# edwardyehuang/iSeg

Hardware: AMD Instinct MI355X
Metric: train_images_per_sec (ConvNeXt-T+ASPP 512x512 crop, fwd+bwd+AdamW, whole job) (higher is better)
Workload: dtype bf16

## Files before the change

### include/iseg_hip.h

```cpp
#ifndef ISEG_HIP_H
#define ISEG_HIP_H

#include <stddef.h>
#include <stdint.h>

#ifdef __cplusplus
extern "C" {
#endif

#ifndef ISEG_HIP_STREAM_T
#define ISEG_HIP_STREAM_T
typedef struct ihipStream_t* iseg_stream_t;
#endif

#define ISEG_STATUS_OK 0
#define ISEG_STATUS_ARG (-1)
#define ISEG_STATUS_HIP (-2)
#define ISEG_STATUS_UNSUPPORTED (-3)
#define ISEG_STATUS_WORKSPACE (-4)

#define ISEG_DTYPE_F32 0
#define ISEG_DTYPE_BF16 1

#define ISEG_ACT_NONE 0
// ... 524 lines not shown

size_t iseg_convnext_mlp_bwd_data_ln_workspace_bytes(int64_t M, int C);
int iseg_convnext_mlp_bwd_data_ln(const void* y1, const float* mean, const float* rstd, const float* ln_gamma, const float* ln_beta,
                                  const void* dout, const float* rowscale, int64_t rows_per_group, const void* bw_tiled, const float* b1,
                                  void* dy1, float* dln_gamma, float* dln_beta, int64_t M, int C, int dtype, void* ws, size_t ws_bytes,
                                  iseg_stream_t stream);
int iseg_convnext_mlp_fwd_ln(const void* y1, const float* ln_gamma, const float* ln_beta, float eps, float* mean, float* rstd,
                             const void* fw_tiled, const float* b1, const float* b2, const float* gamma, const float* rowscale,
                             int64_t rows_per_group, const void* residual, void* out, int64_t M, int C, int dtype, iseg_stream_t stream);
size_t iseg_convnext_mlp_wgrad_workspace_bytes(int64_t M, int C);
int iseg_convnext_mlp_wgrad(const void* y, const float* mean, const float* rstd, const float* ln_gamma, const float* ln_beta,
                            const void* dout, const float* rowscale, int64_t rows_per_group, const void* bw_tiled, const float* b1,
                            const float* W2, const float* b2, const float* gamma, float* dW1, float* db1, float* dW2, float* db2,
                            float* dgamma, int64_t M, int C, int dtype, void* ws, size_t ws_bytes, iseg_stream_t stream);

int iseg_gemma_rope(const void* qkv, int64_t ld_in, void* out, int64_t ld_out, const float* table, int64_t rows, int T, int nq, int nkv, int h,
                    int inverse, int dtype, iseg_stream_t stream);
int iseg_gemma_attention_supported(int nq, int nkv, int h, int dtype);
size_t iseg_gemma_attention_lse_elems(int64_t batch, int T, int nq, int nkv);
int iseg_gemma_attention_fwd(const void* q, int64_t ldq, const void* k, int64_t ldk, const void* v, int64_t ldv, const uint8_t* padding_mask,
                             void* out, int64_t ldo, float* lse2, int64_t batch, int T, int nq, int nkv, int h, float scale, int dtype,
                             iseg_stream_t stream);
int iseg_gemma_attention_bwd(const void* q, int64_t ldq, const void* k, int64_t ldk, const void* v, int64_t ldv, const uint8_t* padding_mask,
                             const void* out, int64_t ldo, const void* dout, int64_t lddo, const float* lse2, float* dsum, void* dq,
                             int64_t lddq, void* dk, int64_t lddk, void* dv, int64_t lddv, int64_t batch, int T, int nq, int nkv, int h,
                             float scale, int dtype, iseg_stream_t stream);
int iseg_embedding_grad(const void* dy, const int64_t* sorted_ids, const int64_t* order, float* dtable, int64_t n, int64_t vocab, int d,
                        float scale, int dtype, iseg_stream_t stream);
int iseg_gemma_rope_cache(const void* qkv, int64_t ld_in, void* q_out, int64_t ldq, void* kcache, int64_t k_batch, int64_t ldk, void* vcache,
                          int64_t v_batch, int64_t ldv, const float* table, int64_t batch, int S, int pos0, int Tn, int nq, int nkv, int h,
// ... 43 lines not shown
```

### iseg_amd/_hip.py

```python
import ctypes as C
import os

_HERE = os.path.dirname(os.path.abspath(__file__))
LIB_PATH = os.path.join(_HERE, "lib", "libiseg_hip.so")

F32, BF16 = 0, 1
ACT_NONE, ACT_RELU, ACT_GELU, ACT_GELU_GRAD, ACT_RELU_GRAD, ACT_MUL_AUX, ACT_SIGMOID, ACT_SWISH, ACT_GELU_TANH = 0, 1, 2, 3, 4, 5, 6, 7, 8
SAMPLE_RANDOM, SAMPLE_TOP_K, SAMPLE_TOP_P = 0, 1, 2
IDS_I32, IDS_I64 = 0, 1


class HipLibraryMissing(RuntimeError):
    pass


class HipCallError(RuntimeError):
    pass


class GemmArgs(C.Structure):
    _fields_ = [
        ("A", C.c_void_p), ("lda", C.c_int64), ("a_kcontig", C.c_int),
        ("B", C.c_void_p), ("ldb", C.c_int64), ("b_kcontig", C.c_int),
        ("D", C.c_void_p), ("ldd", C.c_int64),
# ... 249 lines not shown
    "iseg_conv2d_branches_fwd": (_i, [_p, C.POINTER(ConvBranches), _i, _p, _z, _p]),
    "iseg_conv2d_branches_bwd_data": (_i, [C.POINTER(ConvBranches), _p, _p, _l, _i, _p, _z, _p]),
    "iseg_conv2d_branches_bwd_weight": (_i, [_p, C.POINTER(ConvBranches), _i, _i, _p, _z, _p]),
    "iseg_convnext_mlp_supported": (_i, [_i, _i]),
    "iseg_convnext_mlp_tiled_bytes": (_z, [_i, _i]),
    "iseg_convnext_mlp_prep": (_i, [_p, _p, _p, _p, _p, _i, _p]),
    "iseg_convnext_mlp_fwd": (_i, [_p, _p, _p, _p, _p, _p, _l, _p, _p, _l, _i, _i, _p]),
    "iseg_convnext_mlp_bwd": (_i, [_p, _p, _p, _p, _p, _p, _p, _l, _i, _i, _p]),
    "iseg_convnext_mlp_bwd_data": (_i, [_p, _p, _p, _p, _p, _p, _p, _l, _p, _p, _p, _l, _i, _i, _p]),
    "iseg_convnext_mlp_bwd_data_ln_workspace_bytes": (_z, [_l, _i]),
    "iseg_convnext_mlp_bwd_data_ln": (_i, [_p, _p, _p, _p, _p, _p, _p, _l, _p, _p, _p, _p, _p, _l, _i, _i, _p, _z, _p]),
    "iseg_convnext_weight_prep_batched": (_i, [_p, _i, _l, _p]),
    "iseg_convnext_mlp_fwd_ln": (_i, [_p, _p, _p, _f, _p, _p, _p, _p, _p, _p, _p, _l, _p, _p, _l, _i, _i, _p]),
    "iseg_convnext_mlp_wgrad_workspace_bytes": (_z, [_l, _i]),
    "iseg_convnext_mlp_wgrad": (_i, [_p, _p, _p, _p, _p, _p, _p, _l, _p, _p, _p, _p, _p, _p, _p, _p, _p, _p, _l, _i, _i, _p, _z, _p]),
    "iseg_gemma_rope": (_i, [_p, _l, _p, _l, _p, _l, _i, _i, _i, _i, _i, _i, _p]),
    "iseg_gemma_attention_supported": (_i, [_i, _i, _i, _i]),
    "iseg_gemma_attention_lse_elems": (_z, [_l, _i, _i, _i]),
    "iseg_gemma_attention_fwd": (_i, [_p, _l, _p, _l, _p, _l, _p, _p, _l, _p, _l, _i, _i, _i, _i, _f, _i, _p]),
    "iseg_gemma_attention_bwd": (_i, [_p, _l, _p, _l, _p, _l, _p, _p, _l, _p, _l, _p, _p, _p, _l, _p, _l, _p, _l, _l, _i, _i, _i, _i, _f, _i, _p]),
    "iseg_embedding_grad": (_i, [_p, _p, _p, _p, _l, _l, _i, _f, _i, _p]),
    "iseg_gemma_rope_cache": (_i, [_p, _l, _p, _l, _p, _l, _l, _p, _l, _l, _p, _l, _i, _i, _i, _i, _i, _i, _i, _p]),
    "iseg_gemma_decode_attention_supported": (_i, [_i, _i, _i, _i, _i]),
    "iseg_gemma_decode_attention_splits": (_i, [_l, _i, _i, _i, _i, _i]),
    "iseg_gemma_decode_attention_scratch_bytes": (_z, [_l, _i, _i, _i, _i, _i, _i]),
    "iseg_gemma_decode_attention": (_i, [_p, _l, _p, _l, _l, _p, _l, _l, _p, _l, _p, _z, _l, _i, _i, _i, _i, _i, _i, _f, _i, _i, _p]),
    "iseg_gemma_rope_cache_at": (_i, [_p, _l, _p, _l, _p, _l, _l, _p, _l, _l, _p, _l, _i, _p, _i, _i, _i, _i, _i, _p]),
    "iseg_gemma_decode_attention_at": (_i, [_p, _l, _p, _l, _l, _p, _l, _l, _p, _l, _p, _z, _l, _i, _p, _i, _i, _i, _i, _f, _i, _i, _p]),
    "iseg_decode_commit": (_i, [_p, _l, _p, _l, _p, _p, _p, _p, _l, _i, _l, _i, _i, _p]),
    "iseg_token_sample_supported": (_i, [_l, _i, _i, _i]),
# ... 47 lines not shown
```

### iseg_amd/build.py

```python
import os
import subprocess
import sys
from concurrent.futures import ThreadPoolExecutor

HERE = os.path.dirname(os.path.abspath(__file__))
ROOT = os.path.dirname(HERE)
CSRC = os.path.join(HERE, "csrc")
LIBDIR = os.path.join(HERE, "lib")
LIB = os.path.join(LIBDIR, "libiseg_hip.so")
SOURCES = ["api.hip", "gemm.hip", "gemm_nn.hip", "gemm_nt.hip", "gemm_tn.hip", "norm.hip", "dwconv.hip", "dwconv_mfma.hip", "dwconv_wgrad_mfma.hip", "dwconv_strided.hip", "elementwise.hip", "resize.hip", "loss.hip", "confusion.hip", "ohem.hip", "mask_loss.hip", "sod_metrics.hip", "sod_fmv2.hip", "ccl.hip", "optim.hip", "misc.hip", "attention.hip", "dcnv3.hip", "defattn.hip", "winattn.hip", "flashattn.hip", "selfattn.hip", "mlp_fused.hip", "mlp_wgrad.hip", "conv_igemm.hip", "conv_patchify.hip", "augment.hip", "projective.hip", "grn.hip", "eva.hip", "comm.hip", "mbconv.hip", "sepconv.hip", "jpu.hip", "resblock.hip", "gemma.hip", "gemma_decode.hip", "decode_commit.hip", "token_sample.hip", "lm_head_ce.hip"]
FLAGS = ["--offload-arch=gfx950", "-O3", "-fPIC", "-std=c++17", "-I" + os.path.join(ROOT, "include"), "-I" + CSRC,
         "-Wno-unused-result"] + [f"-D{d}" for d in os.environ.get("ISEG_BUILD_DEFINES", "").split() if d]


def _hipcc():
    for c in (os.environ.get("HIPCC"), "/opt/rocm/bin/hipcc", "hipcc"):
        if c and (os.path.isabs(c) and os.path.exists(c) or not os.path.isabs(c)):
            return c
    raise RuntimeError("hipcc not found")


def _stale(out, deps):
    if not os.path.exists(out):
        return True
    t = os.path.getmtime(out)
# ... 34 lines not shown
```

### iseg_amd/csrc/mlp_wgrad.hip

```cpp
#include "common.h"
#include "iseg_hip.h"
#include "mlp_common.h"

namespace {

typedef __attribute__((address_space(3))) bf16x4* lds_bf16x4_ptr;

template <int C> struct WgGeom {
    static constexpr int WAVES = 8, NT = 64 * WAVES, RT = C > 96 ? 32 : 64;
    static constexpr int HID = 4 * C, KS = C / 32, CBS = C / 16;
    static constexpr int NHG = HID / (16 * WAVES);
    static constexpr int STRIDE = (((2 * C + 223) / 256) * 256 + 32) / 2;
    static constexpr int TILE = RT * STRIDE;
    static constexpr int CPR = C / 8;
    static constexpr int RG = (NT / CPR) >= 32 ? 32 : 16;
    static constexpr int NLOAD = CPR * RG, RPT = RT / RG;
    static constexpr int LDS = 2 * 2 * TILE * 2;
    static constexpr int IMG = C * 64, SLAB = 3 * IMG;
    static_assert(C % 32 == 0 && HID % (16 * WAVES) == 0 && NLOAD <= NT && RT % RG == 0 && LDS <= 160 * 1024, "geometry");
};

__device__ __forceinline__ f32x4 mfma16(const bf16x8& a, const bf16x8& b, const f32x4& c) {
    return __builtin_amdgcn_mfma_f32_16x16x32_bf16(a, b, c, 0, 0, 0);
}

__device__ __forceinline__ bf16x8 tr_frag(const bf16_t* rows, int stride, int cb, int lane) {
    const int q = lane >> 4, qq = (lane >> 2) & 3, p = lane & 3;
    const bf16_t* a0 = rows + (4 * q + qq) * stride + 16 * cb + 4 * p;
    const bf16x4 lo = __builtin_amdgcn_ds_read_tr16_b64_v4bf16((lds_bf16x4_ptr)(a0));
    const bf16x4 hi = __builtin_amdgcn_ds_read_tr16_b64_v4bf16((lds_bf16x4_ptr)(a0 + 16 * stride));
    bf16x8 f;
#pragma unroll
    for (int i = 0; i < 4; ++i) {
        f[i] = lo[i];
        f[4 + i] = hi[i];
    }
    return f;
}

template <int C>
__global__ __launch_bounds__(512) void convnext_mlp_wgrad_kernel(const bf16_t* __restrict__ Y, const float* __restrict__ mean,
                                                                 const float* __restrict__ rstd, const float* __restrict__ ln_gamma,
                                                                 const float* __restrict__ ln_beta, const bf16_t* __restrict__ D,
                                                                 const float* __restrict__ rowscale, int64_t rows_per_group,
                                                                 const void* __restrict__ BW, const float* __restrict__ b1,
                                                                 float* __restrict__ part, int64_t M, int64_t rows_per_chunk, int nchunk) {
    using G = WgGeom<C>;
    constexpr int HID = G::HID, KS = G::KS, CBS = G::CBS, STRIDE = G::STRIDE, TILE = G::TILE, RT = G::RT, RG = G::RG, RPT = G::RPT, CPR = G::CPR;
    extern __shared__ __attribute__((aligned(16))) char smem[];
    bf16_t* const tiles = reinterpret_cast<bf16_t*>(smem);

    const int wg = blockIdx.x, xcd = wg & 7, idx = wg >> 3;
    const int hg = idx % G::NHG, chunk = (idx / G::NHG) * 8 + xcd;
    if (chunk >= nchunk) return;
// ... 196 lines not shown
        v = __builtin_bit_cast(float, (unsigned)sx[0]) + __builtin_bit_cast(float, (unsigned)sx[1]);
        if (lane < 16) pb[hid0 + li] = v;
    }
    if (hg == 0) {
        float* const ss = reinterpret_cast<float*>(smem);
        if (loader) {
#pragma unroll
            for (int u = 0; u < 8; ++u) ss[rg * C + 8 * cpos + u] = s_acc[u];
        }
        __syncthreads();
        if (tid < C) {
            float v = 0.f;
            for (int g = 0; g < RG; ++g) v += ss[g * C + tid];
            ps[tid] = v;
        }
    }
}

constexpr int FIN_ROWS = 8;
__global__ __launch_bounds__(256) void convnext_mlp_wgrad_finish_kernel(const float* __restrict__ rec, const float* __restrict__ W2,
                                                                        const float* __restrict__ b2, const float* __restrict__ gamma,
                                                                        float* __restrict__ dW1, float* __restrict__ db1,
                                                                        float* __restrict__ dW2, float* __restrict__ db2,
                                                                        float* __restrict__ gpart, int C) {
    __shared__ float tw[FIN_ROWS][33];
    __shared__ float tg[8][32];
    const int HID = 4 * C;
    const int c0 = blockIdx.x * 32, h0 = blockIdx.y * FIN_ROWS;
    const int tx = threadIdx.x & 31, ty = threadIdx.x >> 5;
    const int c = c0 + tx;
    const int64_t plane = (int64_t)HID * C;
    const float gm = gamma ? gamma[c] : 1.f;
    {
        const int64_t o = (int64_t)(h0 + ty) * C + c;
        const float z = rec[o], w = rec[plane + o];
        dW2[o] += z * gm;
        tg[ty][tx] = W2[o] * z;
        tw[ty][tx] = w;
    }
    __syncthreads();
    {
        const int hx = threadIdx.x & (FIN_ROWS - 1), cc = threadIdx.x / FIN_ROWS;
        dW1[(int64_t)(c0 + cc) * HID + h0 + hx] += tw[hx][cc];
    }
    if (ty == 0) {
        float v = 0.f;
#pragma unroll
        for (int j = 0; j < 8; ++j) v += tg[j][tx];
        if (blockIdx.y == 0) {
            const float s = rec[2 * plane + HID + c];
            if (gamma) {
                v += b2[c] * s;
                db2[c] += gm * s;
            } else {
                db2[c] += s;
            }
        }
        if (gamma) gpart[(int64_t)blockIdx.y * C + c] = v;
    }
    if (blockIdx.x == 0 && threadIdx.x < FIN_ROWS) {
        const int hid = h0 + threadIdx.x;
        db1[hid] += rec[2 * plane + hid];
    }
}

template <int C> int rows_per_chunk_for(int64_t M, int* nchunk) {
    using G = WgGeom<C>;
    const int target = 8 * (32 / G::NHG);
    int64_t rpc = (M + target - 1) / target;
    rpc = (rpc + 63) / 64 * 64;
    if (rpc < 256) rpc = 256;
    *nchunk = (int)((M + rpc - 1) / rpc);
    return (int)rpc;
}

template <int C>
int launch_wgrad(const void* y, const float* mean, const float* rstd, const float* lng, const float* lnb, const void* d, const float* rowscale,
// ... 14 lines not shown
}

size_t wgrad_ws_floats(int C, int64_t M, int* nchunk_out) {
    int nchunk;
    if (C == 96) rows_per_chunk_for<96>(M, &nchunk);
    else rows_per_chunk_for<192>(M, &nchunk);
    if (nchunk_out) *nchunk_out = nchunk;
    const size_t rec = 2 * 4 * (size_t)C * C + 4 * C + C;
    return (size_t)(nchunk + 1) * rec + (size_t)(4 * C / FIN_ROWS) * C;
}

}

extern "C" size_t iseg_convnext_mlp_wgrad_workspace_bytes(int64_t M, int C) {
    if (!(C == 96 || C == 192) || M <= 0) return 0;
    return wgrad_ws_floats(C, M, nullptr) * sizeof(float);
}

extern "C" int iseg_convnext_mlp_wgrad(const void* y, const float* mean, const float* rstd, const float* ln_gamma, const float* ln_beta,
                                       const void* dout, const float* rowscale, int64_t rows_per_group, const void* bw_tiled, const float* b1,
                                       const float* W2, const float* b2, const float* gamma, float* dW1, float* db1, float* dW2, float* db2,
                                       float* dgamma, int64_t M, int C, int dtype, void* ws, size_t ws_bytes, hipStream_t stream) {
    ISEG_REQUIRE(dtype == ISEG_BF16 && (C == 96 || C == 192), "iseg_convnext_mlp_wgrad: bf16 storage with C = 96 or 192 only (C = %d, dtype = %d)", C, dtype);
    ISEG_REQUIRE(y && dout && bw_tiled && b1 && W2 && b2 && dW1 && db1 && dW2 && db2 && M > 0, "iseg_convnext_mlp_wgrad: null operand or empty problem");
    ISEG_REQUIRE(!gamma || dgamma, "iseg_convnext_mlp_wgrad: gamma needs dgamma");
    ISEG_REQUIRE(!mean || (rstd && ln_gamma && ln_beta), "iseg_convnext_mlp_wgrad: mean needs rstd, ln_gamma and ln_beta");
    ISEG_REQUIRE(!rowscale || (rows_per_group > 0 && rows_per_group % 64 == 0),
                 "iseg_convnext_mlp_wgrad: the row factor must be constant inside 64-row tiles (rows_per_group = %lld)", (long long)rows_per_group);
    ISEG_REQUIRE((((uintptr_t)y | (uintptr_t)dout | (uintptr_t)bw_tiled | (uintptr_t)ln_gamma | (uintptr_t)ln_beta) & 15) == 0,
                 "iseg_convnext_mlp_wgrad: operands must be 16-byte aligned");
    int nchunk;
    const size_t need = wgrad_ws_floats(C, M, &nchunk) * sizeof(float);
    ISEG_NEED_WORKSPACE("iseg_convnext_mlp_wgrad", ws, ws_bytes, need);
    float* const wsf = (float*)ws;
    int rc = C == 96 ? launch_wgrad<96>(y, mean, rstd, ln_gamma, ln_beta, dout, rowscale, rows_per_group, bw_tiled, b1, wsf, M, stream)
                     : launch_wgrad<192>(y, mean, rstd, ln_gamma, ln_beta, dout, rowscale, rows_per_group, bw_tiled, b1, wsf, M, stream);
    if (rc != ISEG_OK) return rc;
    const int HID = 4 * C;
    const int64_t rec = 2 * (int64_t)HID * C + HID + C;
    float* part = wsf;
    float* sum = part + (int64_t)nchunk * rec;
    float* gpart_ws = sum + rec;
    launch_reduce_rows(part, nchunk, rec, 0, 1, rec, sum, nullptr, rec, 0, 1.f, 0, stream);
    const int P = HID / FIN_ROWS;
    float* gpart = gpart_ws;
    float* arena = nullptr;
    if (gamma) {
// ... 12 lines not shown
```

### iseg_amd/functional.py

```python
import math
import os

import torch
from torch.autograd import Function

from . import kernels as K
from . import nn
from . import dist


def _grad(p):
    if p.grad is None:
        p.grad = torch.zeros_like(p.data)
    return p.grad


def _param_grad(p, *shape, scratch=False):
    if p is not None and p.requires_grad:
        g = _grad(p)
    elif p is None or not scratch:
        return None
    else:
        g = torch.zeros(p.shape, dtype=torch.float32, device=p.device)
    return g.reshape(shape) if shape else g
# ... 239 lines not shown
        rpg = M // rowscale.shape[0] if rowscale is not None else 0
        fw, bw = nn.mlp_tiled(W1, W2, None)
        out, mean, rstd = K.convnext_mlp_fwd_ln(x2, ln_gamma.data, ln_beta.data, eps, fw, b1.data, b2.data, None, rowscale, rpg, x2)
        ctx.params, ctx.rpg = (ln_gamma, ln_beta, W1, b1, W2, b2), rpg
        ctx.save_for_backward(x2, mean, rstd, bw, rowscale)
        return out.reshape(x.shape)

    @staticmethod
    def backward(ctx, dout):
        x2, mean, rstd, bw, rowscale = ctx.saved_tensors
        ln_gamma, ln_beta, W1, b1, W2, b2 = ctx.params
        M, C = x2.shape
        do2 = _c(dout).reshape(M, C)
        ln = (mean, rstd, ln_gamma.data, ln_beta.data)
        dx = None
        if ctx.needs_input_grad[0]:
            dln = K.convnext_mlp_bwd_data_ln(x2, do2, bw, b1.data, ln, _grad_out(ln_gamma), _grad_out(ln_beta), rowscale, ctx.rpg)
            dx = K.axpby(do2, dln, 1.0, 1.0, out=dln).reshape(dout.shape)
        else:
            K.convnext_mlp_bwd_data_ln(x2, do2, bw, b1.data, ln, _grad_out(ln_gamma), _grad_out(ln_beta), rowscale, ctx.rpg)
        if any(p.requires_grad for p in (W1, b1, W2, b2)):
            K.convnext_mlp_wgrad(x2, do2, bw, b1.data, W2.data, b2.data, None, _grad_out(W1), _grad_out(b1), _grad_out(W2), _grad_out(b2), None, rowscale,
                                 ctx.rpg, ln=ln)
        dist.grads_ready(ln_gamma, ln_beta, W1, b1, W2, b2)
        return (dx,) + (None,) * 8


def ln_mlp_residual_supported(x, params, drop_path_mask=None):
    ln_gamma, ln_beta, W1, b1, W2, b2 = params
    C = x.shape[-1]
# ... 1253 lines not shown
        ctx.p, ctx.dil, ctx.pad = p, dil, pad
        ctx.save_for_backward(xc, y1, y2, mean, rstd, h, g if grad else None, dp_mask)
        return out.reshape(N, H, W, C)

    @staticmethod
    def backward(ctx, dout):
        xc, y1, y2, mean, rstd, h, g, dp_mask = ctx.saved_tensors
        p, dil, pad = ctx.p, ctx.dil, ctx.pad
        N, H, W, C = xc.shape
        M = N * H * W
        Kk = p.dw_kernel.shape[0]
        do2 = _c(dout).reshape(M, C)
        cdt = xc.dtype
        if ctx.ln_on_load:
            y1m, ln = y1.reshape(M, C), (mean, rstd, p.ln_gamma.data, p.ln_beta.data)
            dy1 = K.convnext_mlp_bwd_data_ln(y1m, do2, h, p.b1.data, ln, _grad_out(p.ln_gamma), _grad_out(p.ln_beta), dp_mask, H * W)
            if any(q is not None and q.requires_grad for q in (p.w1, p.b1, p.w2, p.b2, p.gamma)):
                K.convnext_mlp_wgrad(y1m, do2, h, p.b1.data, p.w2.data, p.b2.data, p.gamma.data if p.gamma is not None else None,
                                     _grad_out(p.w1), _grad_out(p.b1), _grad_out(p.w2), _grad_out(p.b2),
                                     _grad_out(p.gamma) if p.gamma is not None else None, dp_mask, H * W, ln=ln)
            del h
        else:
            dy2 = _ConvNeXtBlockFn._mlp_backward_with_hidden(ctx, p, do2, y2, h, g, dp_mask, H, W, C, M, cdt, xc)
            del h, g
            dy1 = K.layernorm_bwd(dy2, y1.reshape(M, C), p.ln_gamma.data, mean, rstd, _grad_out(p.ln_gamma), _grad_out(p.ln_beta))
        dy1 = dy1.reshape(N, H, W, C)
        if p.dw_kernel.requires_grad or p.dw_bias.requires_grad:
            K.dwconv2d_bwd_weight(xc, dy1, _grad_out(p.dw_kernel, Kk * Kk, C), _grad_out(p.dw_bias), Kk, dil, pad, pad)
        dx = None
        if ctx.needs_input_grad[0]:
            padb = (Kk - 1) * dil - pad
            dx = K.dwconv2d(dy1, p.dw_kernel.data.reshape(Kk * Kk, C), None, Kk, dil, padb, padb, flip=True, add=_c(dout))
# ... 1750 lines not shown
```

### iseg_amd/kernels.py

```python
import contextlib
import ctypes as C

import torch

from . import _hip
from ._hip import F32, BF16, ACT_NONE, ACT_RELU, ACT_GELU, ACT_GELU_GRAD, ACT_RELU_GRAD, ACT_MUL_AUX, ACT_SIGMOID, ACT_SWISH, ACT_GELU_TANH, GemmArgs

_DT = {torch.float32: F32, torch.bfloat16: BF16}


def dt(t):
    try:
        return _DT[t.dtype if isinstance(t, torch.Tensor) else t]
    except KeyError:
        raise TypeError(f"iseg_amd kernels support float32 and bfloat16 storage, got {t.dtype if isinstance(t, torch.Tensor) else t}")


def ptr(t):
    return None if t is None else t.data_ptr()


_DEVICE_INDEX = [None]


# ... 304 lines not shown
    ws, wsb = workspace(need, y1.device)
    _hip.call("iseg_convnext_mlp_bwd_data_ln", ptr(y1), ptr(mean), ptr(rstd), ptr(lng), ptr(lnb), ptr(dout), ptr(rowscale), int(rows_per_group),
              ptr(bw_tiled), ptr(b1), ptr(dy1), ptr(dln_gamma), ptr(dln_beta), M, Cc, dt(y1), ptr(ws), wsb, stream())
    return dy1


def convnext_mlp_wgrad(y, dout, bw_tiled, b1, W2, b2, gamma, dW1, db1, dW2, db2, dgamma, rowscale=None, rows_per_group=0, ln=None):
    _require_cuda(y, dout, bw_tiled)
    M, Cc = y.shape
    need = _hip.lib().iseg_convnext_mlp_wgrad_workspace_bytes(M, Cc)
    ws, wsb = workspace(need, y.device)
    mean, rstd, lng, lnb = ln if ln is not None else (None, None, None, None)
    _hip.call("iseg_convnext_mlp_wgrad", ptr(y), ptr(mean), ptr(rstd), ptr(lng), ptr(lnb), ptr(dout), ptr(rowscale), int(rows_per_group),
              ptr(bw_tiled), ptr(b1), ptr(W2), ptr(b2), ptr(gamma), ptr(dW1), ptr(db1), ptr(dW2), ptr(db2), ptr(dgamma), M, Cc, dt(y), ptr(ws),
              wsb, stream())


def layernorm_fwd(x2d, gamma, beta, eps, save_stats=True):
    _require_cuda(x2d)
    rows, Cc = x2d.shape
    y = torch.empty_like(x2d)
    mean = torch.empty(rows, dtype=torch.float32, device=x2d.device) if save_stats else None
    rstd = torch.empty(rows, dtype=torch.float32, device=x2d.device) if save_stats else None
    _hip.call("iseg_layernorm_fwd", ptr(x2d), ptr(gamma), ptr(beta), ptr(y), ptr(mean), ptr(rstd), rows, Cc, eps, dt(x2d), stream())
    return y, mean, rstd


def layernorm_bwd(dy2d, x2d, gamma, mean, rstd, dgamma, dbeta, dx_add=None, accumulate=True):
    rows, Cc = x2d.shape
    dx = torch.empty_like(x2d)
# ... 1853 lines not shown
```

Baseline: 2103.

## Fuse ConvNeXt MLP data-grad, LayerNorm backward and weight-grad into one pass

Adds a single backward kernel for the C=96 bf16 ConvNeXt MLP. Each row tile is loaded once and the kernel recomputes the hidden activations, produces the input gradient through LayerNorm backward, and accumulates per-chunk W1/W2/bias/LN-parameter partials, which a finish kernel then reduces. Previously the data-grad and weight-grad kernels each re-read the activations and redid the first GEMM. The cost is a large LDS footprint and heavy register use per block, and the path only covers the first stage (C=96).

```diff
diff --git a/include/iseg_hip.h b/include/iseg_hip.h
--- a/include/iseg_hip.h
+++ b/include/iseg_hip.h
@@ -562,6 +562,12 @@
                             const float* W2, const float* b2, const float* gamma, float* dW1, float* db1, float* dW2, float* db2,
                             float* dgamma, int64_t M, int C, int dtype, void* ws, size_t ws_bytes, iseg_stream_t stream);
 
+int iseg_convnext_mlp_bwd_onepass(const void* y1, const float* mean, const float* rstd, const float* ln_gamma, const float* ln_beta,
+                                  const void* dout, const float* rowscale, int64_t rows_per_group, const void* bw_tiled, const float* b1,
+                                  const float* W2, const float* b2, const float* gamma, void* dy1, float* dln_gamma, float* dln_beta,
+                                  float* dW1, float* db1, float* dW2, float* db2, float* dgamma, int64_t M, int C, int dtype, void* ws,
+                                  size_t ws_bytes, iseg_stream_t stream);
+
 int iseg_gemma_rope(const void* qkv, int64_t ld_in, void* out, int64_t ld_out, const float* table, int64_t rows, int T, int nq, int nkv, int h,
                     int inverse, int dtype, iseg_stream_t stream);
 int iseg_gemma_attention_supported(int nq, int nkv, int h, int dtype);
diff --git a/iseg_amd/_hip.py b/iseg_amd/_hip.py
--- a/iseg_amd/_hip.py
+++ b/iseg_amd/_hip.py
@@ -287,6 +287,7 @@
     "iseg_convnext_mlp_fwd_ln": (_i, [_p, _p, _p, _f, _p, _p, _p, _p, _p, _p, _p, _l, _p, _p, _l, _i, _i, _p]),
     "iseg_convnext_mlp_wgrad_workspace_bytes": (_z, [_l, _i]),
     "iseg_convnext_mlp_wgrad": (_i, [_p, _p, _p, _p, _p, _p, _p, _l, _p, _p, _p, _p, _p, _p, _p, _p, _p, _p, _l, _i, _i, _p, _z, _p]),
+    "iseg_convnext_mlp_bwd_onepass": (_i, [_p] * 7 + [_l] + [_p] * 13 + [_l, _i, _i, _p, _z, _p]),
     "iseg_gemma_rope": (_i, [_p, _l, _p, _l, _p, _l, _i, _i, _i, _i, _i, _i, _p]),
     "iseg_gemma_attention_supported": (_i, [_i, _i, _i, _i]),
     "iseg_gemma_attention_lse_elems": (_z, [_l, _i, _i, _i]),
diff --git a/iseg_amd/build.py b/iseg_amd/build.py
--- a/iseg_amd/build.py
+++ b/iseg_amd/build.py
@@ -8,7 +8,7 @@
 CSRC = os.path.join(HERE, "csrc")
 LIBDIR = os.path.join(HERE, "lib")
 LIB = os.path.join(LIBDIR, "libiseg_hip.so")
-SOURCES = ["api.hip", "gemm.hip", "gemm_nn.hip", "gemm_nt.hip", "gemm_tn.hip", "norm.hip", "dwconv.hip", "dwconv_mfma.hip", "dwconv_wgrad_mfma.hip", "dwconv_strided.hip", "elementwise.hip", "resize.hip", "loss.hip", "confusion.hip", "ohem.hip", "mask_loss.hip", "sod_metrics.hip", "sod_fmv2.hip", "ccl.hip", "optim.hip", "misc.hip", "attention.hip", "dcnv3.hip", "defattn.hip", "winattn.hip", "flashattn.hip", "selfattn.hip", "mlp_fused.hip", "mlp_wgrad.hip", "conv_igemm.hip", "conv_patchify.hip", "augment.hip", "projective.hip", "grn.hip", "eva.hip", "comm.hip", "mbconv.hip", "sepconv.hip", "jpu.hip", "resblock.hip", "gemma.hip", "gemma_decode.hip", "decode_commit.hip", "token_sample.hip", "lm_head_ce.hip"]
+SOURCES = ["api.hip", "gemm.hip", "gemm_nn.hip", "gemm_nt.hip", "gemm_tn.hip", "norm.hip", "dwconv.hip", "dwconv_mfma.hip", "dwconv_wgrad_mfma.hip", "dwconv_strided.hip", "elementwise.hip", "resize.hip", "loss.hip", "confusion.hip", "ohem.hip", "mask_loss.hip", "sod_metrics.hip", "sod_fmv2.hip", "ccl.hip", "optim.hip", "misc.hip", "attention.hip", "dcnv3.hip", "defattn.hip", "winattn.hip", "flashattn.hip", "selfattn.hip", "mlp_fused.hip", "mlp_wgrad.hip", "mlp_bwd_onepass.hip", "conv_igemm.hip", "conv_patchify.hip", "augment.hip", "projective.hip", "grn.hip", "eva.hip", "comm.hip", "mbconv.hip", "sepconv.hip", "jpu.hip", "resblock.hip", "gemma.hip", "gemma_decode.hip", "decode_commit.hip", "token_sample.hip", "lm_head_ce.hip"]
 FLAGS = ["--offload-arch=gfx950", "-O3", "-fPIC", "-std=c++17", "-I" + os.path.join(ROOT, "include"), "-I" + CSRC,
          "-Wno-unused-result"] + [f"-D{d}" for d in os.environ.get("ISEG_BUILD_DEFINES", "").split() if d]
 
diff --git a/iseg_amd/csrc/mlp_bwd_onepass.hip b/iseg_amd/csrc/mlp_bwd_onepass.hip
--- /dev/null
+++ b/iseg_amd/csrc/mlp_bwd_onepass.hip
@@ -0,0 +1,401 @@
+#include "common.h"
+#include "iseg_hip.h"
+#include "mlp_common.h"
+#include "mlp_wgrad_common.h"
+
+namespace {
+
+struct OpGeom {
+    static constexpr int C = 96, HID = 4 * C, WAVES = 8, NT = 64 * WAVES, RT = 32, KS = C / 32, CBS = C / 16;
+    static constexpr int NG = HID / (16 * WAVES);
+    static constexpr int YSTR = 144, TILE = RT * YSTR;
+    static constexpr int WSTR = 112;
+    static constexpr int HSTR = HID + 8;
+    static constexpr int DSTR = C + 4;
+    static constexpr int CPR = C / 8, NLOAD = CPR * RT;
+    static constexpr int OFF_W1 = 2 * 2 * TILE * 2;
+    static constexpr int OFF_DH = OFF_W1 + HID * WSTR * 2;
+    static constexpr int OFF_RAW = OFF_DH + RT * HSTR * 2;
+    static constexpr int OFF_ST = OFF_RAW + 2 * RT * C * 2;
+    static constexpr int OFF_LG = OFF_ST + 2 * RT * 2 * 4;
+    static constexpr int LDS = OFF_LG + C * 4;
+    static constexpr int IMG = C * 64, SLAB = 3 * IMG;
+    static constexpr int64_t REC = 2 * (int64_t)HID * C + HID + C;
+    static_assert(NG == 3 && NLOAD <= NT && RT * DSTR * 4 <= 2 * TILE * 2 && 3 * (NT / 32) * C * 4 <= RT * HSTR * 2 && LDS <= 160 * 1024,
+                  "geometry");
+};
+
+__global__ __launch_bounds__(512) void convnext_mlp_bwd_onepass_kernel(const bf16_t* __restrict__ Y, const float* __restrict__ mean,
+                                                                       const float* __restrict__ rstd, const float* __restrict__ ln_gamma,
+                                                                       const float* __restrict__ ln_beta, const bf16_t* __restrict__ D,
+                                                                       const float* __restrict__ rowscale, int64_t rows_per_group,
+                                                                       const void* __restrict__ BW, const float* __restrict__ b1,
+                                                                       bf16_t* __restrict__ DY, float* __restrict__ part,
+                                                                       float* __restrict__ lnpart, int64_t M, int64_t rows_per_chunk) {
+    using G = OpGeom;
+    constexpr int C = G::C, HID = G::HID, KS = G::KS, CBS = G::CBS, NG = G::NG, RT = G::RT, CPR = G::CPR;
+    constexpr int YSTR = G::YSTR, TILE = G::TILE, WSTR = G::WSTR, HSTR = G::HSTR, DSTR = G::DSTR;
+    extern __shared__ __attribute__((aligned(16))) char smem[];
+    bf16_t* const tiles = reinterpret_cast<bf16_t*>(smem);
+    bf16_t* const w1img = reinterpret_cast<bf16_t*>(smem + G::OFF_W1);
+    bf16_t* const dht = reinterpret_cast<bf16_t*>(smem + G::OFF_DH);
+    bf16_t* const raws = reinterpret_cast<bf16_t*>(smem + G::OFF_RAW);
+    float* const stats = reinterpret_cast<float*>(smem + G::OFF_ST);
+    float* const lgs = reinterpret_cast<float*>(smem + G::OFF_LG);
+
+    const int chunk = blockIdx.x;
+    const int tid = threadIdx.x, wid = __builtin_amdgcn_readfirstlane(tid >> 6);
+    auto opaque = [](int v) {
+        asm volatile("" : "+v"(v));
+        return v;
+    };
+    const int64_t r_begin = (int64_t)chunk * rows_per_chunk;
+    const int64_t r_end = r_begin + rows_per_chunk < M ? r_begin + rows_per_chunk : M;
+    const int ntiles = (int)((r_end - r_begin + RT - 1) / RT);
+
+    for (int i = tid; i < HID * CPR; i += G::NT) {
+        const int hid = i / CPR, c8 = i % CPR;
+        const char* src = (const char*)BW + (int64_t)(hid >> 5) * G::SLAB + (c8 >> 1) * 1024 + mlp_frag_offset(hid & 31, c8 & 1);
+        *reinterpret_cast<bf16x8*>(w1img + hid * WSTR + 8 * c8) = *reinterpret_cast<const bf16x8*>(src);
+    }
+    if (tid < C) lgs[tid] = ln_gamma[tid];
+
+    bf16x8 ry, rd;
+    float rmean, rrstd;
+    bool rok;
+    auto issue = [&](int t) {
+        const int tq = opaque(tid);
+        const bool loader = tq < G::NLOAD;
+        const int cpos = tq % CPR, rg = loader ? tq / CPR : 0;
+        const bool live = t < ntiles;
+        const int tt = live ? t : ntiles - 1;
+        const int64_t row = r_begin + (int64_t)tt * RT + rg;
+        const int64_t rr = row < r_end ? row : r_begin;
+        ry = *reinterpret_cast<const bf16x8*>(Y + rr * C + 8 * cpos);
+        rd = *reinterpret_cast<const bf16x8*>(D + rr * C + 8 * cpos);
+        rmean = mean[rr];
+        rrstd = rstd[rr];
+        rok = live && loader && row < r_end;
+    };
+    auto commit = [&](int t, int buf) {
+        const int tq = opaque(tid);
+        const bool loader = tq < G::NLOAD;
+        const int cpos = tq % CPR, rg = loader ? tq / CPR : 0;
+        const int64_t row0 = r_begin + (int64_t)(t < ntiles ? t : ntiles - 1) * RT;
+        const float rs = rowscale ? rowscale[row0 / rows_per_group] : 1.f;
+        float lg[8], lb[8];
+        const int cp = 8 * cpos;
+        load8<float>(ln_gamma + cp, lg);
+        load8<float>(ln_beta + cp, lb);
+        bf16x8 yr = ry, y = ry, d = rd;
+        float mu = rmean, rsd = rrstd;
+        if (!rok) {
+#pragma unroll
+            for (int u = 0; u < 8; ++u) {
+                yr[u] = (bf16_t)0.f;
+                y[u] = (bf16_t)0.f;
+                d[u] = (bf16_t)0.f;
+            }
+            mu = 0.f;
+            rsd = 0.f;
+        } else {
+#pragma unroll
+            for (int u = 0; u < 8; ++u) y[u] = (bf16_t)iseg_ln_apply((float)y[u], mu, rsd, lg[u], lb[u]);
+        }
+        if (rowscale) {
+#pragma unroll
+            for (int u = 0; u < 8; ++u) d[u] = (bf16_t)((float)d[u] * rs);
+        }
+        if (loader) {
+            *reinterpret_cast<bf16x8*>(tiles + (buf * 2 + 0) * TILE + rg * YSTR + 8 * cpos) = y;
+            *reinterpret_cast<bf16x8*>(tiles + (buf * 2 + 1) * TILE + rg * YSTR + 8 * cpos) = d;
+            *reinterpret_cast<bf16x8*>(raws + (buf * RT + rg) * C + 8 * cpos) = yr;
+            if (cpos == 0) {
+                stats[(buf * RT + rg) * 2] = mu;
+                stats[(buf * RT + rg) * 2 + 1] = rsd;
+            }
+        }
+    };
+
+    f32x4 zacc[NG][CBS], wacc[NG][CBS];
+    float db1[NG];
+#pragma unroll
+    for (int g = 0; g < NG; ++g) {
+        db1[g] = 0.f;
+#pragma unroll
+        for (int cb = 0; cb < CBS; ++cb)
+#pragma unroll
+            for (int r = 0; r < 4; ++r) zacc[g][cb][r] = wacc[g][cb][r] = 0.f;
+    }
+
+    float cgs[3], cbs[3], ssum[3];
+#pragma unroll
+    for (int i = 0; i < 3; ++i) cgs[i] = cbs[i] = ssum[i] = 0.f;
+
+    constexpr int CG = 2;
+    bf16x8 w3f[KS];
+    float bias;
+    auto fetch_w3 = [&](int hg) {
+        const int lane = opaque(tid) & 63, li = lane & 15, q = lane >> 4;
+        const char* p = (const char*)BW + (hg >> 1) * G::SLAB + (hg & 1) * 256 + G::IMG + (q >> 1) * 1024 + mlp_frag_offset(li, q & 1);
+#pragma unroll
+        for (int ks = 0; ks < KS; ++ks) w3f[ks] = *reinterpret_cast<const bf16x8*>(p + ks * 2048);
+        bias = b1[hg * 16 + li];
+    };
+    fetch_w3(wid * NG);
+    auto hidden = [&](int t, int buf) {
+        const bf16_t* const ty = tiles + (buf * 2 + 0) * TILE;
+        const bf16_t* const td = tiles + (buf * 2 + 1) * TILE;
+        issue(t + 1);
+#pragma unroll
+        for (int g = 0; g < NG; ++g) {
+            const int hg = wid * NG + g, hid0 = hg * 16;
+            const int lane = opaque(tid) & 63, li = lane & 15, q = lane >> 4;
+            f32x4 hacc[2], dacc[2];
+#pragma unroll
+            for (int b = 0; b < 2; ++b)
+#pragma unroll
+                for (int r = 0; r < 4; ++r) {
+                    hacc[b][r] = bias;
+                    dacc[b][r] = 0.f;
+                }
+#pragma unroll
+            for (int ks = 0; ks < KS; ++ks) {
+                bf16x8 ay[2], ad[2];
+#pragma unroll
+                for (int b = 0; b < 2; ++b) {
+                    const int o = (b * 16 + li) * YSTR + 32 * ks + 8 * q;
+                    ay[b] = *reinterpret_cast<const bf16x8*>(ty + o);
+                    ad[b] = *reinterpret_cast<const bf16x8*>(td + o);
+                }
+                const bf16x8 w1f = *reinterpret_cast<const bf16x8*>(w1img + (hid0 + li) * WSTR + 32 * ks + 8 * q);
+                __builtin_amdgcn_sched_barrier(0);
+#pragma unroll
+                for (int b = 0; b < 2; ++b) {
+                    hacc[b] = mfma16(ay[b], w1f, hacc[b]);
+                    dacc[b] = mfma16(ad[b], w3f[ks], dacc[b]);
+                }
+                __builtin_amdgcn_sched_barrier(0);
+            }
+            fetch_w3(wid * NG + (g + 1) % NG);
+            __builtin_amdgcn_sched_barrier(0);
+            bf16x8 bd[CG], by[CG], gf, hf;
+#pragma unroll
+            for (int b = 0; b < 2; ++b) {
+#pragma unroll
+                for (int r = 0; r < 4; ++r) {
+                    float gl, gd;
+                    gelu_sig_both(hacc[b][r], gl, gd);
+                    const bf16_t dh = (bf16_t)(dacc[b][r] * gd);
+                    gf[4 * b + r] = (bf16_t)gl;
+                    hf[4 * b + r] = dh;
+                    db1[g] += (float)dh;
+                    dht[(16 * b + 4 * q + r) * HSTR + hid0 + li] = dh;
+                }
+                asm volatile("" : "+v"(db1[g]));
+                __builtin_amdgcn_sched_barrier(0);
+                if (b == 0) {
+#pragma unroll
+                    for (int c = 0; c < CG; ++c) {
+                        bd[c] = tr_frag(td, YSTR, c, lane);
+                        by[c] = tr_frag(ty, YSTR, c, lane);
+                    }
+                    __builtin_amdgcn_sched_barrier(0);
+                }
+            }
+#pragma unroll
+            for (int c0 = 0; c0 < CBS; c0 += CG) {
+                if (c0 > 0) {
+#pragma unroll
+                    for (int c = 0; c < CG; ++c) {
+                        bd[c] = tr_frag(td, YSTR, c0 + c, lane);
+                        by[c] = tr_frag(ty, YSTR, c0 + c, lane);
+                    }
+                    __builtin_amdgcn_sched_barrier(0);
+                }
+#pragma unroll
+                for (int c = 0; c < CG; ++c) {
+                    zacc[g][c0 + c] = mfma16(gf, bd[c], zacc[g][c0 + c]);
+                    wacc[g][c0 + c] = mfma16(hf, by[c], wacc[g][c0 + c]);
+                }
+                __builtin_amdgcn_sched_barrier(0);
+            }
+        }
+        const int tq = opaque(tid), hw = tq >> 5, j32 = tq & 31;
+#pragma unroll
+        for (int ps = 0; ps < 2; ++ps)
+#pragma unroll
+            for (int i = 0; i < 3; ++i) ssum[i] += (float)td[(hw + 16 * ps) * YSTR + j32 + 32 * i];
+    };
+
+    auto dy2_tile = [&](int tile, float* dyt) {
+        const int mt = tile & 1, ct = tile >> 1;
+        const int lane = opaque(tid) & 63, li = lane & 15, q = lane >> 4;
+        f32x4 acc;
+#pragma unroll
+        for (int r = 0; r < 4; ++r) acc[r] = 0.f;
+        const bf16_t* const arow = dht + (16 * mt + li) * HSTR + 4 * q;
+#pragma unroll
+        for (int ks = 0; ks < HID / 32; ++ks) {
+            const bf16x4 lo = *reinterpret_cast<const bf16x4*>(arow + 32 * ks);
+            const bf16x4 hi = *reinterpret_cast<const bf16x4*>(arow + 32 * ks + 16);
+            bf16x8 a;
+#pragma unroll
+            for (int i = 0; i < 4; ++i) {
+                a[i] = lo[i];
+                a[4 + i] = hi[i];
+            }
+            acc = mfma16(a, tr_frag(w1img + 32 * ks * WSTR, WSTR, ct, lane), acc);
+            if (ks % 4 == 3) __builtin_amdgcn_sched_barrier(0);
+        }
+#pragma unroll
+        for (int r = 0; r < 4; ++r) dyt[(16 * mt + 4 * q + r) * DSTR + 16 * ct + li] = acc[r];
+    };
+
+    auto layernorm_bwd = [&](int t, int buf, const float* dyt) {
+        const int64_t row0 = r_begin + (int64_t)t * RT;
+        const int tq = opaque(tid), hw = tq >> 5, j32 = tq & 31;
+#pragma unroll
+        for (int ps = 0; ps < 2; ++ps) {
+            const int rr = hw + 16 * ps;
+            const float mu = stats[(buf * RT + rr) * 2], rsd = stats[(buf * RT + rr) * 2 + 1];
+            float v[3], xh[3], tt[3];
+            float s1 = 0.f, s2 = 0.f;
+#pragma unroll
+            for (int i = 0; i < 3; ++i) {
+                v[i] = dyt[rr * DSTR + j32 + 32 * i];
+                xh[i] = ((float)raws[(buf * RT + rr) * C + j32 + 32 * i] - mu) * rsd;
+                tt[i] = v[i] * lgs[j32 + 32 * i];
+                s1 += tt[i];
+                s2 = fmaf(tt[i], xh[i], s2);
+            }
+#pragma unroll
+            for (int o = 16; o > 0; o >>= 1) {
+                s1 += __shfl_xor(s1, o);
+                s2 += __shfl_xor(s2, o);
+            }
+            s1 *= 1.f / (float)C;
+            s2 *= 1.f / (float)C;
+            const int64_t row = row0 + rr;
+            if (row < r_end) {
+#pragma unroll
+                for (int i = 0; i < 3; ++i) DY[row * C + j32 + 32 * i] = (bf16_t)(rsd * (tt[i] - s1 - xh[i] * s2));
+            }
+#pragma unroll
+            for (int i = 0; i < 3; ++i) {
+                cgs[i] = fmaf(v[i], xh[i], cgs[i]);
+                cbs[i] += v[i];
+            }
+        }
+    };
+
+    issue(0);
+    commit(0, 0);
+    __syncthreads();
+    for (int t = 0; t < ntiles; ++t) {
+        const int buf = t & 1;
+        hidden(t, buf);
+        __syncthreads();
+        float* const dyt = reinterpret_cast<float*>(tiles + buf * 2 * TILE);
+        dy2_tile(wid, dyt);
+        if (wid < 4) dy2_tile(8 + wid, dyt);
+        __syncthreads();
+        layernorm_bwd(t, buf, dyt);
+        commit(t + 1, buf ^ 1);
+        __syncthreads();
+    }
+
+    const int lane = tid & 63, li = lane & 15, q = lane >> 4, hw = tid >> 5, j32 = tid & 31;
+    float* const pz = part + (int64_t)chunk * G::REC;
+    float* const pw = pz + (int64_t)HID * C;
+    float* const pb = pw + (int64_t)HID * C;
+    float* const ps = pb + HID;
+#pragma unroll
+    for (int g = 0; g < NG; ++g) {
+        const int hid0 = (wid * NG + g) * 16;
+#pragma unroll
+        for (int cb = 0; cb < CBS; ++cb)
+#pragma unroll
+            for (int r = 0; r < 4; ++r) {
+                const int64_t o = (int64_t)(hid0 + 4 * q + r) * C + 16 * cb + li;
+                pz[o] = zacc[g][cb][r];
+                pw[o] = wacc[g][cb][r];
+            }
+        unsigned u = __builtin_bit_cast(unsigned, db1[g]);
+        auto sw = __builtin_amdgcn_permlane16_swap(u, u, false, false);
+        float v = __builtin_bit_cast(float, (unsigned)sw[0]) + __builtin_bit_cast(float, (unsigned)sw[1]);
+        u = __builtin_bit_cast(unsigned, v);
+        auto sx = __builtin_amdgcn_permlane32_swap(u, u, false, false);
+        v = __builtin_bit_cast(float, (unsigned)sx[0]) + __builtin_bit_cast(float, (unsigned)sx[1]);
+        if (lane < 16) pb[hid0 + li] = v;
+    }
+    float* const ls = reinterpret_cast<float*>(smem + G::OFF_DH);
+#pragma unroll
+    for (int i = 0; i < 3; ++i) {
+        ls[hw * 3 * C + j32 + 32 * i] = ssum[i];
+        ls[hw * 3 * C + C + j32 + 32 * i] = cgs[i];
+        ls[hw * 3 * C + 2 * C + j32 + 32 * i] = cbs[i];
+    }
+    __syncthreads();
+    if (tid < 3 * C) {
+        float v = 0.f;
+        for (int g = 0; g < G::NT / 32; ++g) v += ls[g * 3 * C + tid];
+        if (tid < C) ps[tid] = v;
+        else lnpart[(int64_t)chunk * 2 * C + tid - C] = v;
+    }
+}
+
+}
+
+extern "C" int iseg_convnext_mlp_bwd_onepass(const void* y1, const float* mean, const float* rstd, const float* ln_gamma, const float* ln_beta,
+                                             const void* dout, const float* rowscale, int64_t rows_per_group, const void* bw_tiled,
+                                             const float* b1, const float* W2, const float* b2, const float* gamma, void* dy1,
+                                             float* dln_gamma, float* dln_beta, float* dW1, float* db1, float* dW2, float* db2, float* dgamma,
+                                             int64_t M, int C, int dtype, void* ws, size_t ws_bytes, hipStream_t stream) {
+    using G = OpGeom;
+    ISEG_REQUIRE(dtype == ISEG_BF16 && C == 96, "iseg_convnext_mlp_bwd_onepass: bf16 storage with C = 96 only (C = %d, dtype = %d)", C, dtype);
+    ISEG_REQUIRE(y1 && mean && rstd && ln_gamma && ln_beta && dout && bw_tiled && b1 && W2 && b2 && dy1 && dln_gamma && dln_beta && dW1 && db1 &&
+                     dW2 && db2 && M > 0, "iseg_convnext_mlp_bwd_onepass: null operand or empty problem");
+    ISEG_REQUIRE(!gamma || dgamma, "iseg_convnext_mlp_bwd_onepass: gamma needs dgamma");
+    ISEG_REQUIRE(!rowscale || (rows_per_group > 0 && rows_per_group % 64 == 0),
+                 "iseg_convnext_mlp_bwd_onepass: the row factor must be constant inside 64-row tiles (rows_per_group = %lld)", (long long)rows_per_group);
+    ISEG_REQUIRE((((uintptr_t)y1 | (uintptr_t)dout | (uintptr_t)bw_tiled | (uintptr_t)ln_gamma | (uintptr_t)ln_beta | (uintptr_t)dy1) & 15) == 0,
+                 "iseg_convnext_mlp_bwd_onepass: operands must be 16-byte aligned");
+    int nchunk;
+    const size_t need = iseg_convnext_mlp_wgrad_workspace_bytes(M, C);
+    static_assert(G::REC == 2 * 4 * 96 * 96 + 4 * 96 + 96, "record of onepass_ws_floats");
+    ISEG_NEED_WORKSPACE("iseg_convnext_mlp_bwd_onepass", ws, ws_bytes, need);
+    const int rpc = onepass_rows_per_chunk(M, &nchunk);
+    float* const part = (float*)ws;
+    float* const sum = part + (int64_t)nchunk * G::REC;
+    float* const gpart_ws = sum + G::REC;
+    float* lnpart = gpart_ws + (G::HID / FIN_ROWS) * G::C;
+    float* const ln_arena = iseg_deferred_partials((size_t)nchunk * 2 * G::C * sizeof(float), dln_gamma, dln_beta, 1, stream);
+    if (ln_arena) lnpart = ln_arena;
+    static const bool raised = [] {
+        return hipFuncSetAttribute(reinterpret_cast<const void*>(&convnext_mlp_bwd_onepass_kernel), hipFuncAttributeMaxDynamicSharedMemorySize,
+                                   G::LDS) == hipSuccess;
+    }();
+    (void)raised;
+    hipLaunchKernelGGL(convnext_mlp_bwd_onepass_kernel, dim3(nchunk), dim3(G::NT), G::LDS, stream, (const bf16_t*)y1, mean, rstd, ln_gamma, ln_beta,
+                       (const bf16_t*)dout, rowscale, rows_per_group, bw_tiled, b1, (bf16_t*)dy1, part, lnpart, M, (int64_t)rpc);
+    const int rc = iseg_check_launch("iseg_convnext_mlp_bwd_onepass");
+    if (rc != ISEG_OK) return rc;
+    if (ln_arena) iseg_deferred_push(lnpart, nchunk, 2 * G::C, 2 * G::C, dln_gamma, dln_beta, G::C, 1.f, stream);
+    else launch_reduce_rows(lnpart, nchunk, 2 * G::C, 0, 1, 2 * G::C, dln_gamma, dln_beta, G::C, 0, 1.f, 1, stream);
+    launch_reduce_rows(part, nchunk, G::REC, 0, 1, G::REC, sum, nullptr, G::REC, 0, 1.f, 0, stream);
+    const int P = G::HID / FIN_ROWS;
+    float* gpart = gpart_ws;
+    float* arena = nullptr;
+    if (gamma) {
+        arena = iseg_deferred_partials((size_t)P * G::C * sizeof(float), dgamma, nullptr, 1, stream);
+        if (arena) gpart = arena;
+    }
+    hipLaunchKernelGGL(convnext_mlp_wgrad_finish_kernel, dim3(G::C / 32, G::HID / FIN_ROWS), dim3(256), 0, stream, sum, W2, b2, gamma, dW1, db1, dW2,
+                       db2, gpart, G::C);
+    if (gamma) {
+        if (arena) iseg_deferred_push(gpart, P, G::C, G::C, dgamma, nullptr, G::C, 1.f, stream);
+        else launch_reduce_rows(gpart, P, G::C, 0, 1, G::C, dgamma, nullptr, G::C, 0, 1.f, 1, stream);
+    }
+    return iseg_check_launch("iseg_convnext_mlp_bwd_onepass_finish");
+}
diff --git a/iseg_amd/csrc/mlp_wgrad.hip b/iseg_amd/csrc/mlp_wgrad.hip
--- a/iseg_amd/csrc/mlp_wgrad.hip
+++ b/iseg_amd/csrc/mlp_wgrad.hip
@@ -1,10 +1,9 @@
 #include "common.h"
 #include "iseg_hip.h"
 #include "mlp_common.h"
+#include "mlp_wgrad_common.h"
 
 namespace {
-
-typedef __attribute__((address_space(3))) bf16x4* lds_bf16x4_ptr;
 
 template <int C> struct WgGeom {
     static constexpr int WAVES = 8, NT = 64 * WAVES, RT = C > 96 ? 32 : 64;
@@ -20,24 +19,6 @@
     static_assert(C % 32 == 0 && HID % (16 * WAVES) == 0 && NLOAD <= NT && RT % RG == 0 && LDS <= 160 * 1024, "geometry");
 };
 
-__device__ __forceinline__ f32x4 mfma16(const bf16x8& a, const bf16x8& b, const f32x4& c) {
-    return __builtin_amdgcn_mfma_f32_16x16x32_bf16(a, b, c, 0, 0, 0);
-}
-
-__device__ __forceinline__ bf16x8 tr_frag(const bf16_t* rows, int stride, int cb, int lane) {
-    const int q = lane >> 4, qq = (lane >> 2) & 3, p = lane & 3;
-    const bf16_t* a0 = rows + (4 * q + qq) * stride + 16 * cb + 4 * p;
-    const bf16x4 lo = __builtin_amdgcn_ds_read_tr16_b64_v4bf16((lds_bf16x4_ptr)(a0));
-    const bf16x4 hi = __builtin_amdgcn_ds_read_tr16_b64_v4bf16((lds_bf16x4_ptr)(a0 + 16 * stride));
-    bf16x8 f;
-#pragma unroll
-    for (int i = 0; i < 4; ++i) {
-        f[i] = lo[i];
-        f[4 + i] = hi[i];
-    }
-    return f;
-}
-
 template <int C>
 __global__ __launch_bounds__(512) void convnext_mlp_wgrad_kernel(const bf16_t* __restrict__ Y, const float* __restrict__ mean,
                                                                  const float* __restrict__ rstd, const float* __restrict__ ln_gamma,
@@ -264,53 +245,6 @@
             for (int g = 0; g < RG; ++g) v += ss[g * C + tid];
             ps[tid] = v;
         }
-    }
-}
-
-constexpr int FIN_ROWS = 8;
-__global__ __launch_bounds__(256) void convnext_mlp_wgrad_finish_kernel(const float* __restrict__ rec, const float* __restrict__ W2,
-                                                                        const float* __restrict__ b2, const float* __restrict__ gamma,
-                                                                        float* __restrict__ dW1, float* __restrict__ db1,
-                                                                        float* __restrict__ dW2, float* __restrict__ db2,
-                                                                        float* __restrict__ gpart, int C) {
-    __shared__ float tw[FIN_ROWS][33];
-    __shared__ float tg[8][32];
-    const int HID = 4 * C;
-    const int c0 = blockIdx.x * 32, h0 = blockIdx.y * FIN_ROWS;
-    const int tx = threadIdx.x & 31, ty = threadIdx.x >> 5;
-    const int c = c0 + tx;
-    const int64_t plane = (int64_t)HID * C;
-    const float gm = gamma ? gamma[c] : 1.f;
-    {
-        const int64_t o = (int64_t)(h0 + ty) * C + c;
-        const float z = rec[o], w = rec[plane + o];
-        dW2[o] += z * gm;
-        tg[ty][tx] = W2[o] * z;
-        tw[ty][tx] = w;
-    }
-    __syncthreads();
-    {
-        const int hx = threadIdx.x & (FIN_ROWS - 1), cc = threadIdx.x / FIN_ROWS;
-        dW1[(int64_t)(c0 + cc) * HID + h0 + hx] += tw[hx][cc];
-    }
-    if (ty == 0) {
-        float v = 0.f;
-#pragma unroll
-        for (int j = 0; j < 8; ++j) v += tg[j][tx];
-        if (blockIdx.y == 0) {
-            const float s = rec[2 * plane + HID + c];
-            if (gamma) {
-                v += b2[c] * s;
-                db2[c] += gm * s;
-            } else {
-                db2[c] += s;
-            }
-        }
-        if (gamma) gpart[(int64_t)blockIdx.y * C + c] = v;
-    }
-    if (blockIdx.x == 0 && threadIdx.x < FIN_ROWS) {
-        const int hid = h0 + threadIdx.x;
-        db1[hid] += rec[2 * plane + hid];
     }
 }
 
@@ -355,7 +289,9 @@
 
 extern "C" size_t iseg_convnext_mlp_wgrad_workspace_bytes(int64_t M, int C) {
     if (!(C == 96 || C == 192) || M <= 0) return 0;
-    return wgrad_ws_floats(C, M, nullptr) * sizeof(float);
+    size_t floats = wgrad_ws_floats(C, M, nullptr);
+    if (C == 96 && onepass_ws_floats(M, nullptr) > floats) floats = onepass_ws_floats(M, nullptr);
+    return floats * sizeof(float);
 }
 
 extern "C" int iseg_convnext_mlp_wgrad(const void* y, const float* mean, const float* rstd, const float* ln_gamma, const float* ln_beta,
@@ -371,7 +307,8 @@
     ISEG_REQUIRE((((uintptr_t)y | (uintptr_t)dout | (uintptr_t)bw_tiled | (uintptr_t)ln_gamma | (uintptr_t)ln_beta) & 15) == 0,
                  "iseg_convnext_mlp_wgrad: operands must be 16-byte aligned");
     int nchunk;
-    const size_t need = wgrad_ws_floats(C, M, &nchunk) * sizeof(float);
+    wgrad_ws_floats(C, M, &nchunk);
+    const size_t need = iseg_convnext_mlp_wgrad_workspace_bytes(M, C);
     ISEG_NEED_WORKSPACE("iseg_convnext_mlp_wgrad", ws, ws_bytes, need);
     float* const wsf = (float*)ws;
     int rc = C == 96 ? launch_wgrad<96>(y, mean, rstd, ln_gamma, ln_beta, dout, rowscale, rows_per_group, bw_tiled, b1, wsf, M, stream)
diff --git a/iseg_amd/csrc/mlp_wgrad_common.h b/iseg_amd/csrc/mlp_wgrad_common.h
--- /dev/null
+++ b/iseg_amd/csrc/mlp_wgrad_common.h
@@ -0,0 +1,90 @@
+#pragma once
+#include "common.h"
+
+namespace {
+
+typedef __attribute__((address_space(3))) bf16x4* lds_bf16x4_ptr;
+
+__device__ __forceinline__ f32x4 mfma16(const bf16x8& a, const bf16x8& b, const f32x4& c) {
+    return __builtin_amdgcn_mfma_f32_16x16x32_bf16(a, b, c, 0, 0, 0);
+}
+
+__device__ __forceinline__ bf16x8 tr_frag(const bf16_t* rows, int stride, int cb, int lane) {
+    const int q = lane >> 4, qq = (lane >> 2) & 3, p = lane & 3;
+    const bf16_t* a0 = rows + (4 * q + qq) * stride + 16 * cb + 4 * p;
+    const bf16x4 lo = __builtin_amdgcn_ds_read_tr16_b64_v4bf16((lds_bf16x4_ptr)(a0));
+    const bf16x4 hi = __builtin_amdgcn_ds_read_tr16_b64_v4bf16((lds_bf16x4_ptr)(a0 + 16 * stride));
+    bf16x8 f;
+#pragma unroll
+    for (int i = 0; i < 4; ++i) {
+        f[i] = lo[i];
+        f[4 + i] = hi[i];
+    }
+    return f;
+}
+
+constexpr int FIN_ROWS = 8;
+__global__ __launch_bounds__(256) void convnext_mlp_wgrad_finish_kernel(const float* __restrict__ rec, const float* __restrict__ W2,
+                                                                        const float* __restrict__ b2, const float* __restrict__ gamma,
+                                                                        float* __restrict__ dW1, float* __restrict__ db1,
+                                                                        float* __restrict__ dW2, float* __restrict__ db2,
+                                                                        float* __restrict__ gpart, int C) {
+    __shared__ float tw[FIN_ROWS][33];
+    __shared__ float tg[8][32];
+    const int HID = 4 * C;
+    const int c0 = blockIdx.x * 32, h0 = blockIdx.y * FIN_ROWS;
+    const int tx = threadIdx.x & 31, ty = threadIdx.x >> 5;
+    const int c = c0 + tx;
+    const int64_t plane = (int64_t)HID * C;
+    const float gm = gamma ? gamma[c] : 1.f;
+    {
+        const int64_t o = (int64_t)(h0 + ty) * C + c;
+        const float z = rec[o], w = rec[plane + o];
+        dW2[o] += z * gm;
+        tg[ty][tx] = W2[o] * z;
+        tw[ty][tx] = w;
+    }
+    __syncthreads();
+    {
+        const int hx = threadIdx.x & (FIN_ROWS - 1), cc = threadIdx.x / FIN_ROWS;
+        dW1[(int64_t)(c0 + cc) * HID + h0 + hx] += tw[hx][cc];
+    }
+    if (ty == 0) {
+        float v = 0.f;
+#pragma unroll
+        for (int j = 0; j < 8; ++j) v += tg[j][tx];
+        if (blockIdx.y == 0) {
+            const float s = rec[2 * plane + HID + c];
+            if (gamma) {
+                v += b2[c] * s;
+                db2[c] += gm * s;
+            } else {
+                db2[c] += s;
+            }
+        }
+        if (gamma) gpart[(int64_t)blockIdx.y * C + c] = v;
+    }
+    if (blockIdx.x == 0 && threadIdx.x < FIN_ROWS) {
+        const int hid = h0 + threadIdx.x;
+        db1[hid] += rec[2 * plane + hid];
+    }
+}
+
+inline int onepass_rows_per_chunk(int64_t M, int* nchunk) {
+    int64_t rpc = (M + 255) / 256;
+    rpc = (rpc + 63) / 64 * 64;
+    if (rpc < 256) rpc = 256;
+    *nchunk = (int)((M + rpc - 1) / rpc);
+    return (int)rpc;
+}
+
+inline size_t onepass_ws_floats(int64_t M, int* nchunk_out) {
+    constexpr int C = 96, HID = 4 * C;
+    constexpr size_t REC = 2 * (size_t)HID * C + HID + C;
+    int nchunk;
+    onepass_rows_per_chunk(M, &nchunk);
+    if (nchunk_out) *nchunk_out = nchunk;
+    return (size_t)(nchunk + 1) * REC + (size_t)(HID / FIN_ROWS) * C + (size_t)nchunk * 2 * C;
+}
+
+}
diff --git a/iseg_amd/functional.py b/iseg_amd/functional.py
--- a/iseg_amd/functional.py
+++ b/iseg_amd/functional.py
@@ -277,6 +277,13 @@
         do2 = _c(dout).reshape(M, C)
         ln = (mean, rstd, ln_gamma.data, ln_beta.data)
         dx = None
+        if K.convnext_mlp_bwd_onepass_supported(C, x2.dtype) and any(p.requires_grad for p in (W1, b1, W2, b2)):
+            dln = K.convnext_mlp_bwd_onepass(x2, do2, bw, b1.data, W2.data, b2.data, None, ln, _grad_out(ln_gamma), _grad_out(ln_beta),
+                                             _grad_out(W1), _grad_out(b1), _grad_out(W2), _grad_out(b2), None, rowscale, ctx.rpg)
+            if ctx.needs_input_grad[0]:
+                dx = K.axpby(do2, dln, 1.0, 1.0, out=dln).reshape(dout.shape)
+            dist.grads_ready(ln_gamma, ln_beta, W1, b1, W2, b2)
+            return (dx,) + (None,) * 8
         if ctx.needs_input_grad[0]:
             dln = K.convnext_mlp_bwd_data_ln(x2, do2, bw, b1.data, ln, _grad_out(ln_gamma), _grad_out(ln_beta), rowscale, ctx.rpg)
             dx = K.axpby(do2, dln, 1.0, 1.0, out=dln).reshape(dout.shape)
@@ -1560,8 +1567,15 @@
         cdt = xc.dtype
         if ctx.ln_on_load:
             y1m, ln = y1.reshape(M, C), (mean, rstd, p.ln_gamma.data, p.ln_beta.data)
-            dy1 = K.convnext_mlp_bwd_data_ln(y1m, do2, h, p.b1.data, ln, _grad_out(p.ln_gamma), _grad_out(p.ln_beta), dp_mask, H * W)
-            if any(q is not None and q.requires_grad for q in (p.w1, p.b1, p.w2, p.b2, p.gamma)):
+            mlp_grads = any(q is not None and q.requires_grad for q in (p.w1, p.b1, p.w2, p.b2, p.gamma))
+            if mlp_grads and K.convnext_mlp_bwd_onepass_supported(C, cdt):
+                dy1 = K.convnext_mlp_bwd_onepass(y1m, do2, h, p.b1.data, p.w2.data, p.b2.data, p.gamma.data if p.gamma is not None else None, ln,
+                                                 _grad_out(p.ln_gamma), _grad_out(p.ln_beta), _grad_out(p.w1), _grad_out(p.b1), _grad_out(p.w2),
+                                                 _grad_out(p.b2), _grad_out(p.gamma) if p.gamma is not None else None, dp_mask, H * W)
+                mlp_grads = False
+            else:
+                dy1 = K.convnext_mlp_bwd_data_ln(y1m, do2, h, p.b1.data, ln, _grad_out(p.ln_gamma), _grad_out(p.ln_beta), dp_mask, H * W)
+            if mlp_grads:
                 K.convnext_mlp_wgrad(y1m, do2, h, p.b1.data, p.w2.data, p.b2.data, p.gamma.data if p.gamma is not None else None,
                                      _grad_out(p.w1), _grad_out(p.b1), _grad_out(p.w2), _grad_out(p.b2),
                                      _grad_out(p.gamma) if p.gamma is not None else None, dp_mask, H * W, ln=ln)
diff --git a/iseg_amd/kernels.py b/iseg_amd/kernels.py
--- a/iseg_amd/kernels.py
+++ b/iseg_amd/kernels.py
@@ -342,6 +342,24 @@
     _hip.call("iseg_convnext_mlp_wgrad", ptr(y), ptr(mean), ptr(rstd), ptr(lng), ptr(lnb), ptr(dout), ptr(rowscale), int(rows_per_group),
               ptr(bw_tiled), ptr(b1), ptr(W2), ptr(b2), ptr(gamma), ptr(dW1), ptr(db1), ptr(dW2), ptr(db2), ptr(dgamma), M, Cc, dt(y), ptr(ws),
               wsb, stream())
+
+
+def convnext_mlp_bwd_onepass_supported(C, dtype):
+    return C == 96 and dtype == torch.bfloat16
+
+
+def convnext_mlp_bwd_onepass(y1, dout, bw_tiled, b1, W2, b2, gamma, ln, dln_gamma, dln_beta, dW1, db1, dW2, db2, dgamma, rowscale=None,
+                             rows_per_group=0):
+    _require_cuda(y1, dout, bw_tiled, dln_gamma, dln_beta)
+    M, Cc = y1.shape
+    dy1 = torch.empty((M, Cc), dtype=y1.dtype, device=y1.device)
+    mean, rstd, lng, lnb = ln
+    need = _hip.lib().iseg_convnext_mlp_wgrad_workspace_bytes(M, Cc)
+    ws, wsb = workspace(need, y1.device)
+    _hip.call("iseg_convnext_mlp_bwd_onepass", ptr(y1), ptr(mean), ptr(rstd), ptr(lng), ptr(lnb), ptr(dout), ptr(rowscale), int(rows_per_group),
+              ptr(bw_tiled), ptr(b1), ptr(W2), ptr(b2), ptr(gamma), ptr(dy1), ptr(dln_gamma), ptr(dln_beta), ptr(dW1), ptr(db1), ptr(dW2),
+              ptr(db2), ptr(dgamma), M, Cc, dt(y1), ptr(ws), wsb, stream())
+    return dy1
 
 
 def layernorm_fwd(x2d, gamma, beta, eps, save_stats=True):
```

After: 2138 (median of 6 runs). +1.7%, better.
